# wq2012/SpectralCluster

Measured on AMD Instinct MI355X. Metric: predict() calls/sec, n=8192 d=256 ICASSP2018 (GraphCut, eigengap k in [2,20], cosine k-means), higher is better.
Workload: dtype f64; 1 GPU; icassp2018_graphcut_n8192_d256_k8_max20; n_samples=8192, n_features=256, parallelism=replicas x1, collectives=none

## Files before the change

### spectralcluster_amd/csrc/gemm_f64.hip

```cpp
#include <algorithm>
#include <cstdio>
#include <cstdlib>
#include <type_traits>
#include <vector>

#include <cstring>

#include "sc_internal.h"

namespace sc {

typedef double v4f64 __attribute__((ext_vector_type(4)));
typedef int v4i32 __attribute__((ext_vector_type(4)));
typedef double v2f64 __attribute__((ext_vector_type(2)));

constexpr int BM = 128;
constexpr int BN = 128;
constexpr int BK = 16;

__device__ __forceinline__ int lds_chunk_off(int row, int kc) {
  return row * BK + ((2 * kc) ^ (row & 14));
}

template <bool SYM>
__device__ __forceinline__ void tile_coords(int id, int ntiles_m, int ntiles_n,
                                            int* ti, int* tj) {
  if (SYM) {
    int r = 0, rowlen = ntiles_m;
    while (id >= rowlen) {
      id -= rowlen;
      --rowlen;
      ++r;
    }
    *ti = r;
    *tj = r + id;
  } else {
    *ti = id / ntiles_n;
    *tj = id - (*ti) * ntiles_n;
  }
}

struct GemmStats {
  double* pmax;
  double* psum;
  int mode;
  const double* addend;
};

template <int EPI, bool SYM>
__device__ __forceinline__ void tile_row_stats(const v4f64 (&acc)[4][4], int ti, int tj,
                                               int ntiles, int M, int N, int tid,
                                               const GemmStats& st, double* scratch) {
  const int lane = tid & 63, wave = tid >> 6;
  const int wr = wave >> 1, wc = wave & 1;
  const int li = lane & 15, lg = lane >> 4;
  double* rmax = scratch;
  double* rsum = scratch + 256;
  double* cmax = scratch + 512;
  double* csum = scratch + 768;
  const bool diag_tile = ti == tj;
#pragma unroll
  for (int m = 0; m < 4; ++m) {
#pragma unroll
    for (int r = 0; r < 4; ++r) {
      const int lrow = wr * 64 + m * 16 + lg + 4 * r;
      double mx = -INFINITY, sm = 0.0;
#pragma unroll
      for (int nn = 0; nn < 4; ++nn) {
        const int lcol = wc * 64 + nn * 16 + li;
        const bool inside = tj * BN + lcol < N;
        const bool skip = st.mode == 2 && diag_tile && lrow == lcol;
        double x = acc[m][nn][r];
        if (EPI == kEpiAffinity) x = __builtin_fma(x, 0.5, 0.5);
        if (inside && !skip) mx = fmax(mx, x);
        if (inside) sm += x;
      }
#pragma unroll
      for (int o = 1; o < 16; o <<= 1) {
        mx = fmax(mx, __shfl_xor(mx, o));
        sm += __shfl_xor(sm, o);
      }
      if (li == 0) {
        rmax[wc * 128 + lrow] = mx;
        rsum[wc * 128 + lrow] = sm;
      }
      __builtin_amdgcn_sched_barrier(0);
    }
  }
  if (SYM && !diag_tile) {
#pragma unroll
    for (int nn = 0; nn < 4; ++nn) {
      const int lcol = wc * 64 + nn * 16 + li;
      double mx = -INFINITY, sm = 0.0;
#pragma unroll
      for (int m = 0; m < 4; ++m)
#pragma unroll
        for (int r = 0; r < 4; ++r) {
          const int lrow = wr * 64 + m * 16 + lg + 4 * r;
          double x = acc[m][nn][r];
          if (EPI == kEpiAffinity) x = __builtin_fma(x, 0.5, 0.5);
          if (ti * BM + lrow < M) {
            mx = fmax(mx, x);
            sm += x;
          }
        }
      mx = fmax(mx, __shfl_xor(mx, 16));
      sm += __shfl_xor(sm, 16);
      mx = fmax(mx, __shfl_xor(mx, 32));
      sm += __shfl_xor(sm, 32);
      if (lg == 0) {
        cmax[wr * 128 + lcol] = mx;
        csum[wr * 128 + lcol] = sm;
      }
      __builtin_amdgcn_sched_barrier(0);
    }
  }
  __syncthreads();
  if (tid < 128) {
    const int row = ti * BM + tid;
    if (row < M) {
      st.pmax[(size_t)row * ntiles + tj] = fmax(rmax[tid], rmax[128 + tid]);
      if (st.mode == 1) st.psum[(size_t)row * ntiles + tj] = rsum[tid] + rsum[128 + tid];
    }
  } else if (SYM && !diag_tile) {
    const int c = tid - 128;
    const int row = tj * BN + c;
    if (row < N) {
      st.pmax[(size_t)row * ntiles + ti] = fmax(cmax[c], cmax[128 + c]);
      if (st.mode == 1) st.psum[(size_t)row * ntiles + ti] = csum[c] + csum[128 + c];
    }
  }
}

__device__ __forceinline__ double vmax64(double a, double b) {
  double d;
  asm("v_max_f64 %0, %1, %2" : "=v"(d) : "v"(a), "v"(b));
  return d;
}

constexpr int kEpiColPart = 1024;
constexpr int kEpiStage = 3072;
constexpr int kEpiStageWave = 1280;
constexpr int kEpiRowPitch = 17;

template <int EPI, bool SYM>
__device__ __forceinline__ void tile_row_stats_full(const v4f64 (&acc)[4][4], int ti, int tj,
                                                    int ntiles, int tid, const GemmStats& st,
                                                    double* smem) {
  const int lane = tid & 63, wave = tid >> 6;
  const int wr = wave >> 1, wc = wave & 1;
  const int li = lane & 15, lg = lane >> 4;
  const bool diag_tile = ti == tj;
  const bool sums = st.mode == 1;
  const bool crop = st.mode == 2 && diag_tile && wr == wc;
  double* rmax = smem;
  double* rsum = smem + 256;
  double* cpart = smem + kEpiColPart;
  double* T = smem + kEpiStage + wave * (64 * kEpiRowPitch);
  auto el = [&](int m, int nn, int r) -> double {
    const double x = acc[m][nn][r];
    return EPI == kEpiAffinity ? __builtin_fma(x, 0.5, 0.5) : x;
  };
  auto rows_of = [&](auto is_sum) {
    constexpr bool SUM = decltype(is_sum)::value;
#pragma unroll
    for (int m = 0; m < 4; ++m)
#pragma unroll
      for (int r = 0; r < 4; ++r) {
        double a[4];
#pragma unroll
        for (int nn = 0; nn < 4; ++nn) a[nn] = el(m, nn, r);
        double v;
        if (SUM) {
          v = (a[0] + a[1]) + (a[2] + a[3]);
        } else {
          if (crop && lg + 4 * r == li) a[m] = -INFINITY;
          v = vmax64(vmax64(a[0], a[1]), vmax64(a[2], a[3]));
        }
        T[(m * 16 + lg + 4 * r) * kEpiRowPitch + li] = v;
      }
    __builtin_amdgcn_fence(__ATOMIC_RELEASE, "wavefront");
    __builtin_amdgcn_wave_barrier();
    double t[16];
#pragma unroll
    for (int j = 0; j < 16; ++j) t[j] = T[lane * kEpiRowPitch + j];
#pragma unroll
    for (int w = 8; w >= 1; w >>= 1)
#pragma unroll
      for (int j = 0; j < w; ++j) t[j] = SUM ? t[j] + t[j + w] : vmax64(t[j], t[j + w]);
    (SUM ? rsum : rmax)[wc * 128 + wr * 64 + lane] = t[0];
    __builtin_amdgcn_fence(__ATOMIC_ACQUIRE, "wavefront");
    __builtin_amdgcn_wave_barrier();
  };
  rows_of(std::false_type{});
  if (sums) rows_of(std::true_type{});
  const bool mirror = SYM && !diag_tile;
  if (mirror) {
#pragma unroll
    for (int nn = 0; nn < 4; ++nn) {
      double mx[4], sm[4];
#pragma unroll
      for (int m = 0; m < 4; ++m) {
        const double x0 = el(m, nn, 0), x1 = el(m, nn, 1), x2 = el(m, nn, 2), x3 = el(m, nn, 3);
        mx[m] = vmax64(vmax64(x0, x1), vmax64(x2, x3));
        sm[m] = (x0 + x1) + (x2 + x3);
      }
      const int slot = (wr * 4 + lg) * 128 + wc * 64 + nn * 16 + li;
      cpart[slot] = vmax64(vmax64(mx[0], mx[1]), vmax64(mx[2], mx[3]));
      if (sums) cpart[1024 + slot] = (sm[0] + sm[1]) + (sm[2] + sm[3]);
    }
  }
  __syncthreads();
  if (tid < 128) {
    const size_t at = (size_t)(ti * BM + tid) * ntiles + tj;
    st.pmax[at] = vmax64(rmax[tid], rmax[128 + tid]);
    if (sums) st.psum[at] = rsum[tid] + rsum[128 + tid];
  } else if (mirror) {
    const int c = tid - 128;
    const size_t at = (size_t)(tj * BN + c) * ntiles + ti;
    double t[8];
#pragma unroll
    for (int j = 0; j < 8; ++j) t[j] = cpart[j * 128 + c];
    st.pmax[at] = vmax64(vmax64(vmax64(t[0], t[1]), vmax64(t[2], t[3])),
                         vmax64(vmax64(t[4], t[5]), vmax64(t[6], t[7])));
    if (sums) {
#pragma unroll
      for (int j = 0; j < 8; ++j) t[j] = cpart[1024 + j * 128 + c];
      st.psum[at] = ((t[0] + t[1]) + (t[2] + t[3])) + ((t[4] + t[5]) + (t[6] + t[7]));
    }
  }
}

__global__ void k_gemm_stats_reduce(const double* __restrict__ pmax,
                                    const double* __restrict__ psum, int n, int ntiles,
                                    int mode, double* __restrict__ rowmax,
                                    double* __restrict__ rowsum) {
  const int i = blockIdx.x * blockDim.x + threadIdx.x;
  if (i >= n) return;
  double mx = -INFINITY, sm = 0.0;
  for (int t = 0; t < ntiles; ++t) {
    mx = fmax(mx, pmax[(size_t)i * ntiles + t]);
    if (mode == 1) sm += psum[(size_t)i * ntiles + t];
  }
  if (mode == 2) mx = fmax(mx, 0.0);
  rowmax[i] = mx;
  if (mode == 1) rowsum[i] = sm;
}

constexpr int kStatRows = 32;
constexpr int kStatMaxTiles = 120;
__device__ __forceinline__ void gemm_stats_reduce_lds_body(
    const double* __restrict__ pmax, const double* __restrict__ psum, int n, int ntiles, int mode,
    double* __restrict__ rowmax, double* __restrict__ rowsum) {
  extern __shared__ __attribute__((aligned(16))) double st_smem[];
  const int pitch = ntiles + 1;
  double* lmax = st_smem;
  double* lsum = st_smem + kStatRows * pitch;
  const int r0 = blockIdx.x * kStatRows;
  const int rows = min(kStatRows, n - r0);
  const int total = rows * ntiles;
  for (int e = threadIdx.x; e < total; e += blockDim.x) {
    const int rr = e / ntiles, t = e - rr * ntiles;
    lmax[rr * pitch + t] = pmax[(size_t)r0 * ntiles + e];
    if (mode == 1) lsum[rr * pitch + t] = psum[(size_t)r0 * ntiles + e];
  }
  __syncthreads();
  if ((int)threadIdx.x >= rows) return;
  double mx = -INFINITY, sm = 0.0;
  for (int t = 0; t < ntiles; ++t) {
    mx = fmax(mx, lmax[threadIdx.x * pitch + t]);
    if (mode == 1) sm += lsum[threadIdx.x * pitch + t];
  }
  if (mode == 2) mx = fmax(mx, 0.0);
  rowmax[r0 + threadIdx.x] = mx;
  if (mode == 1) rowsum[r0 + threadIdx.x] = sm;
}
__global__ __launch_bounds__(256) void k_gemm_stats_reduce_lds(
    const double* __restrict__ pmax, const double* __restrict__ psum, int n, int ntiles, int mode,
    double* __restrict__ rowmax, double* __restrict__ rowsum) {
  gemm_stats_reduce_lds_body(pmax, psum, n, ntiles, mode, rowmax, rowsum);
}

struct GemmMember {
  const double* A;
  double* C;
  double* pmax;
  double* psum;
  const int2* tilemap;
  int lda, ldc, n, K, nt;
};
struct GemmGroup {
  GemmMember m[kGroupMax];
  int first[kGroupMax + 1];
};
struct GemmPairMember {
  const double* A;
  const double* B;
  const double* addend;
  double* C;
  const int2* tilemap;
  int lda, ldb, ldc, n, nt;
};
struct GemmPairGroup {
  GemmPairMember m[kGroupMax];
  int first[kGroupMax + 1];
};

constexpr int kEdgePrio = 3;

template <int EPI, bool SYM, bool GROUPED, class GRP>
__device__ __forceinline__ void gemm_nt_body(const double* __restrict__ A,
                                                 int lda,
                                                 const double* __restrict__ B,
                                                 int ldb, double* __restrict__ C,
                                                 int ldc, int M, int N, int K,
                                                 int ntiles_m, int ntiles_n,
                                                 int full_tiles, int ksplit_tail,
                                                 double* __restrict__ partial,
                                                 double* __restrict__ probe_out,
                                                 const int2* __restrict__ tilemap,
                                                 int xcd_chunk, GemmStats stats,
                                                 int* __restrict__ queue,
                                                 int nunits, int persist,
                                                 const GRP* __restrict__ grp) {
  __shared__ __attribute__((aligned(16))) double smem[2 * BM * BK + 2 * BN * BK];
  double(*As)[BM * BK] = reinterpret_cast<double(*)[BM * BK]>(smem);
  double(*Bs)[BN * BK] = reinterpret_cast<double(*)[BN * BK]>(smem + 2 * BM * BK);

  for (int iter = 0;; ++iter) {
  if (iter > 0) {
    if (GROUPED || !persist || queue == nullptr) break;
    __syncthreads();
  }
  if (kEdgePrio & 1) __builtin_amdgcn_s_setprio(3);
  int ti, tj;
  int item_blk = (int)blockIdx.x;
  if constexpr (GROUPED) {
    item_blk = (item_blk & 7) * xcd_chunk + (item_blk >> 3);
    if (item_blk >= grp->first[kGroupMax]) continue;
    int z = 0;
    while (item_blk >= grp->first[z + 1]) ++z;
    const auto& g = grp->m[z];
    item_blk -= grp->first[z];
    C = g.C;
    ldc = g.ldc;
    M = N = g.n;
    ntiles_m = ntiles_n = g.nt;
    tilemap = g.tilemap;
    if constexpr (std::is_same<GRP, GemmPairGroup>::value) {
      A = g.A;
      B = g.B;
      lda = g.lda;
      ldb = g.ldb;
      K = g.n;
      stats.addend = g.addend;
    } else {
      A = B = g.A;
      lda = ldb = g.lda;
      K = g.K;
      stats.pmax = g.pmax;
      stats.psum = g.psum;
    }
  }
  if (queue != nullptr) {
    int* s_item = reinterpret_cast<int*>(smem);
    if (threadIdx.x == 0) {
      const int x = (int)blockIdx.x & 7;
      auto draw = [&](int* counter, int limit) -> int {
        if (__hip_atomic_load(counter, __ATOMIC_RELAXED, __HIP_MEMORY_SCOPE_AGENT) >= limit)
          return -1;
        const int v = __hip_atomic_fetch_add(counter, 1, __ATOMIC_RELAXED,
                                             __HIP_MEMORY_SCOPE_AGENT);
        return v < limit ? v : -1;
      };
      int got = -1;
      {
        const int k = draw(&queue[x], xcd_chunk);
        if (k >= 0) got = x + 8 * k;
      }
      if (got < 0) {
        const int u = draw(&queue[9], nunits);
        if (u >= 0) got = full_tiles + u;
      }
      for (int dx = 1; got < 0 && dx < 8; ++dx) {
        const int xx = (x + dx) & 7;
        const int k = draw(&queue[xx], xcd_chunk);
        if (k >= 0) got = xx + 8 * k;
      }
      *s_item = got;
    }
    __syncthreads();
    item_blk = *s_item;
    __syncthreads();
    if (item_blk < 0) break;
  }
  const bool whole = item_blk < full_tiles;
  const int unit = whole ? 0 : item_blk - full_tiles;
  const int ksplit = whole ? 1 : ksplit_tail;
  const int chunk = unit % ksplit;
  int tile = whole ? item_blk : full_tiles + unit / ksplit;
  if (!GROUPED && whole && xcd_chunk > 0) tile = (tile & 7) * xcd_chunk + (tile >> 3);
  if (!whole) stats.mode = 0;
  if (tilemap != nullptr) {
    const int2 t = tilemap[tile];
    ti = t.x;
    tj = t.y;
  } else {
    tile_coords<SYM>(tile, ntiles_m, ntiles_n, &ti, &tj);
  }
  const int row0 = ti * BM;
  const int col0 = tj * BN;

  int tid_ = threadIdx.x;
  asm volatile("" : "+v"(tid_));
  const int tid = tid_;
  const int lane = tid & 63;
  const int wave = tid >> 6;
  const int wr = wave >> 1;
  const int wc = wave & 1;
  const int li = lane & 15;
  const int lg = lane >> 4;
  long long clk0 = 0, wall0 = 0;
  const bool probe = whole && probe_out != nullptr;
  if (probe) {
    clk0 = clock64();
    wall0 = wall_clock64();
  }
// ... 10 lines not shown
    boff[q] = (unsigned)(((size_t)rb_ * ldb + 2 * kc0) * sizeof(double));
    lds_off[q] = lds_chunk_off(r, kc0);
  }

  v4f64 acc[4][4];
#pragma unroll
  for (int m = 0; m < 4; ++m)
#pragma unroll
    for (int nn = 0; nn < 4; ++nn) acc[m][nn] = (v4f64){0.0, 0.0, 0.0, 0.0};

  const int ktiles_all = (K + BK - 1) / BK;
  const int kper = (ktiles_all + ksplit - 1) / ksplit;
  const int kt_begin = chunk * kper;
  const int kt_end = min(ktiles_all, kt_begin + kper);
  double2 ra[4], rb[4];

  const __amdgpu_buffer_rsrc_t arsrc =
      __builtin_amdgcn_make_buffer_rsrc(const_cast<double*>(A + (size_t)row0 * lda), 0, -1,
                                        0x00020000);
  const __amdgpu_buffer_rsrc_t brsrc =
      __builtin_amdgcn_make_buffer_rsrc(const_cast<double*>(B + (size_t)col0 * ldb), 0, -1,
                                        0x00020000);
  auto gload = [&](int kt) {
    const int koff = kt * BK * (int)sizeof(double);
#pragma unroll
    for (int q = 0; q < 4; ++q) {
      const v4i32 va = __builtin_amdgcn_raw_buffer_load_b128(arsrc, aoff[q], koff, 0);
      const v4i32 vb = __builtin_amdgcn_raw_buffer_load_b128(brsrc, boff[q], koff, 0);
      ra[q] = __builtin_bit_cast(double2, va);
      rb[q] = __builtin_bit_cast(double2, vb);
    }
  };

  auto lds_store = [&](int buf, int kt) {
    const int k0 = kt * BK;
    if (k0 + BK > K) {
      const int k = k0 + 2 * kc0;
#pragma unroll
      for (int q = 0; q < 4; ++q) {
        if (k >= K) { ra[q].x = 0.0; rb[q].x = 0.0; }
        if (k + 1 >= K) { ra[q].y = 0.0; rb[q].y = 0.0; }
      }
    }
#pragma unroll
    for (int q = 0; q < 4; ++q) {
      *reinterpret_cast<double2*>(&As[buf][lds_off[q]]) = ra[q];
      *reinterpret_cast<double2*>(&Bs[buf][lds_off[q]]) = rb[q];
    }
  };

  const int arow = (wr * 64 + li) * BK;
  const int brow = (wc * 64 + li) * BK;

  const int first_buf = (__builtin_amdgcn_s_getreg(6 | (31 << 11)) & 0xfff) != 0 ? 1 : 0;
  if (kt_begin < kt_end) {
    gload(kt_begin);
    lds_store(first_buf, kt_begin);
    if (kt_begin + 1 < kt_end) gload(kt_begin + 1);
  }
  __syncthreads();

  double2 fa0[4], fb0[4], fa1[4], fb1[4];
  auto load_frags = [&](double2 (&a)[4], double2 (&b)[4], const double* Ac, const double* Bc,
                        int p) {
    const int koff = (2 * (4 * p + lg)) ^ (li & 14);
#pragma unroll
    for (int m = 0; m < 4; ++m)
      a[m] = *reinterpret_cast<const double2*>(Ac + arow + m * 16 * BK + koff);
#pragma unroll
    for (int nn = 0; nn < 4; ++nn)
      b[nn] = *reinterpret_cast<const double2*>(Bc + brow + nn * 16 * BK + koff);
  };
  auto mfma16x = [&](const double2 (&a)[4], const double2 (&b)[4]) {
#pragma unroll
    for (int m = 0; m < 4; ++m)
#pragma unroll
      for (int nn = 0; nn < 4; ++nn)
        acc[m][nn] = __builtin_amdgcn_mfma_f64_16x16x4f64(a[m].x, b[nn].x, acc[m][nn], 0, 0, 0);
  };
  auto mfma16y = [&](const double2 (&a)[4], const double2 (&b)[4]) {
#pragma unroll
    for (int m = 0; m < 4; ++m)
#pragma unroll
      for (int nn = 0; nn < 4; ++nn)
        acc[m][nn] = __builtin_amdgcn_mfma_f64_16x16x4f64(a[m].y, b[nn].y, acc[m][nn], 0, 0, 0);
  };
  if (kt_begin < kt_end) load_frags(fa0, fb0, As[first_buf], Bs[first_buf], 0);
  auto k_tile = [&](int kt, auto cur_c, auto prio_c) {
    constexpr int cur = decltype(cur_c)::value;
    constexpr int prio = decltype(prio_c)::value;
    load_frags(fa1, fb1, As[cur], Bs[cur], 1);
    __builtin_amdgcn_sched_barrier(0);
    __builtin_amdgcn_s_setprio(prio);
    mfma16x(fa0, fb0);
    __builtin_amdgcn_sched_barrier(0);
    if (kt + 1 < kt_end) {
      lds_store(cur ^ 1, kt + 1);
      if (kt + 2 < kt_end) gload(kt + 2);
    }
    __builtin_amdgcn_sched_barrier(0);
    mfma16y(fa0, fb0);
    __builtin_amdgcn_s_setprio(0);
    __builtin_amdgcn_sched_barrier(0);
    __syncthreads();
    if (kt + 1 < kt_end) load_frags(fa0, fb0, As[cur ^ 1], Bs[cur ^ 1], 0);
    __builtin_amdgcn_sched_barrier(0);
    __builtin_amdgcn_s_setprio(prio);
    mfma16x(fa1, fb1);
    mfma16y(fa1, fb1);
    __builtin_amdgcn_s_setprio(0);
    __builtin_amdgcn_sched_barrier(0);
  };
  long long wall_k0 = 0;
  if (probe) wall_k0 = wall_clock64();
  {
    using P0 = std::integral_constant<int, 2>;
    using P1 = std::integral_constant<int, 1>;
    int kt = kt_begin;
    if (first_buf && kt < kt_end) {
      k_tile(kt, std::integral_constant<int, 1>{}, P1{});
      ++kt;
    }
    for (; kt + 1 < kt_end; kt += 2) {
      k_tile(kt, std::integral_constant<int, 0>{}, P0{});
      k_tile(kt + 1, std::integral_constant<int, 1>{}, P1{});
    }
    if (kt < kt_end) k_tile(kt, std::integral_constant<int, 0>{}, P0{});
  }

  if (kEdgePrio & 1) __builtin_amdgcn_s_setprio(3);
  long long wall_k1 = 0;
  if (probe) wall_k1 = wall_clock64();
  if (probe && tid == 0) {
    probe_out[2 * item_blk] = (double)(clock64() - clk0);
    probe_out[2 * item_blk + 1] = (double)(wall_k1 - wall0);
    probe_out[2 * full_tiles + item_blk] = (double)wall0;
    probe_out[3 * full_tiles + item_blk] = (double)(wall_k0 - wall0);
  }
  if (ksplit > 1) {
    double* out = partial + (size_t)unit * (BM * BN);
#pragma unroll
    for (int m = 0; m < 4; ++m)
#pragma unroll
      for (int nn = 0; nn < 4; ++nn)
#pragma unroll
        for (int r = 0; r < 4; ++r)
          out[((m * 4 + nn) * 4 + r) * 256 + tid] = acc[m][nn][r];
    continue;
  }
  const bool mirror = SYM && (ti != tj);
  constexpr bool nt_store = (kEdgePrio & 2) != 0;
  const bool full = row0 + BM <= M && col0 + BN <= N;
  if (stats.mode != 0 || mirror) __syncthreads();
  if (stats.mode != 0) {
    if (full) tile_row_stats_full<EPI, SYM>(acc, ti, tj, ntiles_n, tid, stats, smem);
    else tile_row_stats<EPI, SYM>(acc, ti, tj, ntiles_n, M, N, tid, stats, smem);
    __builtin_amdgcn_sched_barrier(0);
  }
  if (probe && tid == 0) probe_out[4 * full_tiles + item_blk] = (double)(wall_clock64() - wall_k1);
  constexpr int kStagePitch = 20;
  double* stage = smem + kEpiStage + wave * kEpiStageWave;
  if (full) {
    double* cdir = C + (size_t)(row0 + wr * 64 + lg) * ldc + (col0 + wc * 64 + li);
    const double* adir = nullptr;
    if (EPI == kEpiAdd)
      adir = stats.addend + (size_t)(row0 + wr * 64 + lg) * ldc + (col0 + wc * 64 + li);
    double* cmir = C + (size_t)(col0 + wc * 64 + (lane >> 3)) * ldc + (row0 + wr * 64 + 2 * (lane & 7));
    double* stage_w = stage + li * kStagePitch + lg;
    const double* stage_r = stage + (lane >> 3) * kStagePitch + 2 * (lane & 7);
    auto store_full = [&](auto mirror_c) {
      constexpr bool MIRROR = decltype(mirror_c)::value;
#pragma unroll
      for (int m = 0; m < 4; ++m) {
#pragma unroll
        for (int r = 0; r < 4; ++r) {
          const size_t roff = (size_t)(m * 16 + 4 * r) * ldc;
#pragma unroll
          for (int nn = 0; nn < 4; ++nn) {
            double v = acc[m][nn][r];
            if (EPI == kEpiAffinity) v = __builtin_fma(v, 0.5, 0.5);
            if (EPI == kEpiAdd) v += adir[roff + nn * 16];
            if (nt_store) __builtin_nontemporal_store(v, cdir + roff + nn * 16);
            else cdir[roff + nn * 16] = v;
            if (MIRROR) stage_w[nn * 16 * kStagePitch + 4 * r] = v;
          }
        }
        if (MIRROR) {
          __builtin_amdgcn_fence(__ATOMIC_RELEASE, "wavefront");
          __builtin_amdgcn_wave_barrier();
#pragma unroll
          for (int i = 0; i < 8; ++i) {
            const v2f64 v = *reinterpret_cast<const v2f64*>(stage_r + i * 8 * kStagePitch);
            v2f64* dst = reinterpret_cast<v2f64*>(cmir + (size_t)(i * 8) * ldc + m * 16);
            if (nt_store) __builtin_nontemporal_store(v, dst);
            else *dst = v;
          }
          __builtin_amdgcn_fence(__ATOMIC_ACQUIRE, "wavefront");
          __builtin_amdgcn_wave_barrier();
        }
      }
    };
    if (mirror) store_full(std::true_type{});
    else store_full(std::false_type{});
  } else {
#pragma unroll
  for (int m = 0; m < 4; ++m) {
#pragma unroll
    for (int nn = 0; nn < 4; ++nn) {
      const int col = col0 + wc * 64 + nn * 16 + li;
#pragma unroll
      for (int r = 0; r < 4; ++r) {
        const int row = row0 + wr * 64 + m * 16 + lg + 4 * r;
        double v = acc[m][nn][r];
        if (EPI == kEpiAffinity) v = __builtin_fma(v, 0.5, 0.5);
        if (row < M && col < N) {
          if (EPI == kEpiAdd) v += stats.addend[(size_t)row * ldc + col];
          if (nt_store) __builtin_nontemporal_store(v, &C[(size_t)row * ldc + col]);
          else C[(size_t)row * ldc + col] = v;
        }
        if (mirror) stage[(nn * 16 + li) * kStagePitch + lg + 4 * r] = v;
      }
    }
    if (mirror) {
      __builtin_amdgcn_fence(__ATOMIC_RELEASE, "wavefront");
      __builtin_amdgcn_wave_barrier();
#pragma unroll
      for (int i = 0; i < 8; ++i) {
        const int c = i * 8 + (lane >> 3);
        const int j = 2 * (lane & 7);
        const double2 v = *reinterpret_cast<const double2*>(stage + c * kStagePitch + j);
        const int mrow = col0 + wc * 64 + c;
        const int mcol = row0 + wr * 64 + m * 16 + j;
        if (mrow < N) {
          double* dst = C + (size_t)mrow * ldc + mcol;
          if (mcol + 1 < M) {
            if (nt_store) {
              __builtin_nontemporal_store(v.x, dst);
              __builtin_nontemporal_store(v.y, dst + 1);
            } else {
              *reinterpret_cast<double2*>(dst) = v;
            }
          } else if (mcol < M) {
            dst[0] = v.x;
          }
        }
      }
      __builtin_amdgcn_fence(__ATOMIC_ACQUIRE, "wavefront");
      __builtin_amdgcn_wave_barrier();
    }
  }
  }
  if (probe) {
    const long long t_issued = wall_clock64();
    asm volatile("s_waitcnt vmcnt(0)" ::: "memory");
    if (tid == 0) {
      probe_out[5 * full_tiles + item_blk] = (double)(t_issued - wall_k1);
      probe_out[6 * full_tiles + item_blk] = (double)(wall_clock64() - wall_k1);
    }
  }
  }
}

template <int EPI, bool SYM>
__global__ __launch_bounds__(256, 2) void k_gemm_nt(const double* __restrict__ A,
                                                 int lda,
                                                 const double* __restrict__ B,
                                                 int ldb, double* __restrict__ C,
                                                 int ldc, int M, int N, int K,
                                                 int ntiles_m, int ntiles_n,
                                                 int full_tiles, int ksplit_tail,
                                                 double* __restrict__ partial,
                                                 double* __restrict__ probe_out,
                                                 const int2* __restrict__ tilemap,
                                                 int xcd_chunk, GemmStats stats,
                                                 int* __restrict__ queue,
                                                 int nunits, int persist) {
  gemm_nt_body<EPI, SYM, false, GemmGroup>(A, lda, B, ldb, C, ldc, M, N, K, ntiles_m, ntiles_n,
                                           full_tiles, ksplit_tail, partial, probe_out, tilemap,
                                           xcd_chunk, stats, queue, nunits, persist, nullptr);
}
template <int EPI>
__global__ __launch_bounds__(256, 2) void k_gemm_nt_g(const GemmGroup grp, int stats_mode,
                                                     int xcd_chunk) {
  GemmStats stats{nullptr, nullptr, stats_mode, nullptr};
  gemm_nt_body<EPI, true, true, GemmGroup>(nullptr, 0, nullptr, 0, nullptr, 0, 0, 0, 0, 0, 0,
                                           0x7fffffff, 1, nullptr, nullptr, nullptr, xcd_chunk,
                                           stats, nullptr, 0, 0, &grp);
}
template <int EPI>
__global__ __launch_bounds__(256, 2) void k_gemm_nt_pg(const GemmPairGroup grp, int xcd_chunk) {
  GemmStats stats{nullptr, nullptr, 0, nullptr};
  gemm_nt_body<EPI, true, true, GemmPairGroup>(nullptr, 0, nullptr, 0, nullptr, 0, 0, 0, 0, 0, 0,
                                               0x7fffffff, 1, nullptr, nullptr, nullptr,
                                               xcd_chunk, stats, nullptr, 0, 0, &grp);
}
template <int EPI>
__global__ __launch_bounds__(256, 2) void k_gemm_nt_pgf(const GemmPairGroup grp, int xcd_chunk) {
  GemmStats stats{nullptr, nullptr, 0, nullptr};
  gemm_nt_body<EPI, false, true, GemmPairGroup>(nullptr, 0, nullptr, 0, nullptr, 0, 0, 0, 0, 0, 0,
                                                0x7fffffff, 1, nullptr, nullptr, nullptr,
                                                xcd_chunk, stats, nullptr, 0, 0, &grp);
}

struct StatsReduceItem {
  const double* pmax;
  const double* psum;
  double* rowmax;
  double* rowsum;
  int n, nt;
};
__global__ __launch_bounds__(256) void k_gemm_stats_reduce_g(const GroupOf<StatsReduceItem> g,
                                                             int mode) {
  const StatsReduceItem& a = g.s[blockIdx.y];
  if ((int)blockIdx.x * kStatRows >= a.n) return;
  if (a.nt > kStatMaxTiles) {
    const int i = blockIdx.x * kStatRows + threadIdx.x;
    if ((int)threadIdx.x >= kStatRows || i >= a.n) return;
    double mx, sm;
    gemm_stats_fold_row(a.pmax + (size_t)i * a.nt,
                        mode == 1 ? a.psum + (size_t)i * a.nt : nullptr, a.nt, mode, &mx, &sm);
    a.rowmax[i] = mx;
    if (mode == 1) a.rowsum[i] = sm;
    return;
  }
  gemm_stats_reduce_lds_body(a.pmax, a.psum, a.n, a.nt, mode, a.rowmax, a.rowsum);
}

template <int EPI, bool SYM>
__global__ __launch_bounds__(256) void k_gemm_reduce(const double* __restrict__ partial,
                                                     double* __restrict__ C, int ldc,
                                                     int M, int N, int ntiles_m,
                                                     int ntiles_n, int tile_offset,
                                                     int ksplit,
                                                     const int2* __restrict__ tilemap,
                                                     const double* __restrict__ addend) {
  int ti, tj;
  if (tilemap != nullptr) {
    const int2 t = tilemap[tile_offset + blockIdx.x];
    ti = t.x;
    tj = t.y;
  } else {
    tile_coords<SYM>(tile_offset + blockIdx.x, ntiles_m, ntiles_n, &ti, &tj);
  }
  const int tid = threadIdx.x;
  const int lane = tid & 63, wave = tid >> 6;
  const int wr = wave >> 1, wc = wave & 1;
  const int li = lane & 15, lg = lane >> 4;
  const bool mirror = SYM && (ti != tj);
  const double* base = partial + (size_t)blockIdx.x * ksplit * (BM * BN);
  {
    const int m = blockIdx.y >> 2;
    {
      const int nn = blockIdx.y & 3;
      const int col = tj * BN + wc * 64 + nn * 16 + li;
#pragma unroll
      for (int r = 0; r < 4; ++r) {
        const int row = ti * BM + wr * 64 + m * 16 + lg + 4 * r;
        const int slot = ((m * 4 + nn) * 4 + r) * 256 + tid;
        double v = 0.0;
        for (int c = 0; c < ksplit; ++c) v += base[(size_t)c * (BM * BN) + slot];
        if (EPI == kEpiAffinity) v = __builtin_fma(v, 0.5, 0.5);
        if (row < M && col < N) {
          if (EPI == kEpiAdd) v += addend[(size_t)row * ldc + col];
          C[(size_t)row * ldc + col] = v;
          if (mirror) C[(size_t)col * ldc + row] = v;
        }
      }
    }
  }
}

template <bool SYM>
__global__ __launch_bounds__(256) void k_gemm_tail_stats(const double* __restrict__ C, int ldc,
                                                         int M, int N, int ntiles_m,
                                                         int ntiles_n, int tile_base,
                                                         const int2* __restrict__ tilemap,
                                                         GemmStats st) {
  int ti, tj;
  if (tilemap != nullptr) {
    const int2 t = tilemap[tile_base + blockIdx.x];
    ti = t.x;
    tj = t.y;
  } else {
    tile_coords<SYM>(tile_base + blockIdx.x, ntiles_m, ntiles_n, &ti, &tj);
  }
  if (blockIdx.y == 1) {
    if (!SYM || ti == tj) return;
    const int t = ti;
    ti = tj;
    tj = t;
  }
  const int lane = threadIdx.x & 63, wave = threadIdx.x >> 6;
  for (int lr = blockIdx.z * 16 + wave; lr < blockIdx.z * 16 + 16; lr += 4) {
    const int row = ti * BM + lr;
    if (row >= M) break;
    double mx = -INFINITY, sm = 0.0;
#pragma unroll
    for (int h = 0; h < 2; ++h) {
      const int col = tj * BN + lane + 64 * h;
      if (col < N) {
        const double x = C[(size_t)row * ldc + col];
        if (!(st.mode == 2 && row == col)) mx = fmax(mx, x);
        sm += x;
      }
    }
#pragma unroll
    for (int o = 1; o < 64; o <<= 1) {
      mx = fmax(mx, __shfl_xor(mx, o));
      sm += __shfl_xor(sm, o);
    }
    if (lane == 0) {
      st.pmax[(size_t)row * ntiles_n + tj] = mx;
      if (st.mode == 1) st.psum[(size_t)row * ntiles_n + tj] = sm;
    }
  }
}

__global__ void k_gemm_queue_init(int* queue) { queue[threadIdx.x] = 0; }

int gemm_resident_slots() {
  static int slots_dev[16] = {0};
  int dev = 0;
  hipGetDevice(&dev);
  dev = dev < 16 ? dev : 0;
  if (slots_dev[dev] == 0) {
    int per_cu = 0;
    hipDeviceProp_t prop;
    hipGetDeviceProperties(&prop, dev);
    hipOccupancyMaxActiveBlocksPerMultiprocessor(
        &per_cu, reinterpret_cast<const void*>(k_gemm_nt<kEpiNone, true>), 256, 0);
    if (per_cu < 1) per_cu = 1;
    slots_dev[dev] = per_cu * prop.multiProcessorCount;
  }
  return slots_dev[dev];
}
constexpr int kQueueWords = 16;
size_t gemm_splitk_workspace_bytes() {
  return (size_t)gemm_resident_slots() * BM * BN * sizeof(double) + kQueueWords * sizeof(int);
}

template <int EPI, bool SYM>
static void launch_variant(hipStream_t s, const double* A, int lda, const double* B,
                           int ldb, double* C, int ldc, int M, int N, int K,
                           double* splitk_ws, const int2* tilemap, const GemmRowStats* rs,
                           const double* addend) {
  GemmStats stats{nullptr, nullptr, 0, addend};
  if (rs != nullptr && rs->mode != 0) {
    stats.pmax = rs->partial_max;
    stats.psum = rs->partial_sum;
    stats.mode = rs->mode;
  }
  const int tm = (M + BM - 1) / BM;
  const int tn = (N + BN - 1) / BN;
  const int tiles = SYM ? tm * (tm + 1) / 2 : tm * tn;
  const int g_slots = gemm_resident_slots();
  double* g_partial = splitk_ws;
  const int ktiles = (K + BK - 1) / BK;
  int full = (tiles / g_slots) * g_slots;
  int rem = tiles - full;
  int ksplit = 1;
  if (rem > 0) {
    if (splitk_ws != nullptr) {
      ksplit = g_slots / rem;
      ksplit = std::min(ksplit, std::max(1, ktiles / 8));
      if (K <= 512 && full == 0) ksplit = 1;
    }
    if (ksplit < 2) {
      full = tiles;
      rem = 0;
      ksplit = 1;
    }
  }
  {
    const int xcd_chunk = (tilemap != nullptr && full % 8 == 0 && full >= 512) ? full / 8 : 0;
    static double* dbg = nullptr;
    static const char* probe_env = getenv("SC_GEMM_CLOCK");
    if (probe_env != nullptr && dbg == nullptr) (void)hipMalloc(&dbg, sizeof(double) * 7 * 8192);
    double* probe = (full > 0 && full <= 8192) ? dbg : nullptr;
    int* queue = nullptr;
    if (K >= 1024 && xcd_chunk > 0 && rem > 0 && SYM) {
      queue = reinterpret_cast<int*>(splitk_ws + (size_t)g_slots * BM * BN);
      hipLaunchKernelGGL(k_gemm_queue_init, dim3(1), dim3(kQueueWords), 0, s, queue);
    }
    const int persist = queue != nullptr ? 1 : 0;
    const int grid = persist ? std::min(g_slots, full + rem * ksplit) : full + rem * ksplit;
    hipLaunchKernelGGL((k_gemm_nt<EPI, SYM>), dim3(grid), dim3(256), 0, s, A, lda,
                       B, ldb, C, ldc, M, N, K, tm, tn, full, ksplit, g_partial, probe, tilemap,
                       xcd_chunk, stats, queue, rem * ksplit, persist);
    if (probe != nullptr) {
      (void)hipStreamSynchronize(s);
      std::vector<double> h(7 * full);
      (void)hipMemcpy(h.data(), dbg, sizeof(double) * 7 * full, hipMemcpyDeviceToHost);
      if (strcmp(probe_env, "1") != 0) {
        const char* path = probe_env;
        if (FILE* f = fopen(path, "w")) {
          for (int b = 0; b < full; ++b)
            fprintf(f, "%d %.0f %.0f %.0f %.0f %.0f %.0f %.0f\n", b, h[2 * b], h[2 * b + 1],
                    h[2 * full + b], h[3 * full + b], h[4 * full + b], h[5 * full + b],
                    h[6 * full + b]);
          fclose(f);
        }
      }
      double c = 0, w = 0;
      for (int i = 0; i < full; ++i) { c += h[2 * i]; w += h[2 * i + 1]; }
      int rate = 0;
      (void)hipDeviceGetAttribute(&rate, hipDeviceAttributeWallClockRate, 0);
      fprintf(stderr, "gemm clock probe (epilogue %d%s): %d tiles, K %d, shader cycles/tile %.0f "
              "(MFMA-bound minimum %.0f), effective shader clock %.1f MHz, tile time %.1f us\n",
              EPI, SYM ? ", symmetric" : "", full, K, c / full,
              (double)((K + BK - 1) / BK) * 64 * 64 * 2, c / w * rate / 1e3,
              w / full / rate * 1e3);
    }
  }
  if (rem > 0) {
    hipLaunchKernelGGL((k_gemm_reduce<EPI, SYM>), dim3(rem, 16), dim3(256), 0, s, g_partial,
                       C, ldc, M, N, tm, tn, full, ksplit, tilemap, addend);
    if (stats.mode != 0)
      hipLaunchKernelGGL((k_gemm_tail_stats<SYM>), dim3(rem, SYM ? 2 : 1, 8), dim3(256), 0, s, C,
                         ldc, M, N, tm, tn, full, tilemap, stats);
  }
  if (stats.mode != 0) {
    if (tn <= kStatMaxTiles)
      hipLaunchKernelGGL(k_gemm_stats_reduce_lds, dim3((M + kStatRows - 1) / kStatRows), dim3(256),
                         2 * kStatRows * (size_t)(tn + 1) * sizeof(double), s, stats.pmax,
                         stats.psum, M, tn, stats.mode, rs->rowmax, rs->rowsum);
    else
      hipLaunchKernelGGL(k_gemm_stats_reduce, dim3((M + 255) / 256), dim3(256), 0, s, stats.pmax,
                         stats.psum, M, tn, stats.mode, rs->rowmax, rs->rowsum);
  }
}

void gemm_build_sym_tilemap(int nt, std::vector<int2>* out) {
  out->clear();
  const int np = (nt + 7) / 8;
  for (int pi = 0; pi < np; ++pi)
    for (int pj = pi; pj < np; ++pj)
      for (int ti = pi * 8; ti < std::min(nt, pi * 8 + 8); ++ti)
        for (int tj = std::max(ti, pj * 8); tj < std::min(nt, pj * 8 + 8); ++tj)
          out->push_back(make_int2(ti, tj));
}
int gemm_tile_dim(int n) { return (n + BM - 1) / BM; }

void launch_gemm_nt(hipStream_t s, const double* A, int lda, const double* B,
                    int ldb, double* C, int ldc, int M, int N, int K,
                    int epilogue, bool symmetric, double* splitk_ws,
                    const int2* tilemap, const GemmRowStats* rs, const double* addend) {
  if (M <= 0 || N <= 0) return;
#define SC_GEMM_CASE(E, S)                                                                \
  launch_variant<E, S>(s, A, lda, B, ldb, C, ldc, M, N, K, splitk_ws, S ? tilemap : nullptr, \
                       rs, addend)
  if (symmetric) {
    if (epilogue == kEpiAffinity) SC_GEMM_CASE(kEpiAffinity, true);
    else if (epilogue == kEpiAdd) SC_GEMM_CASE(kEpiAdd, true);
    else SC_GEMM_CASE(kEpiNone, true);
  } else {
    if (epilogue == kEpiAffinity) SC_GEMM_CASE(kEpiAffinity, false);
    else if (epilogue == kEpiAdd) SC_GEMM_CASE(kEpiAdd, false);
    else SC_GEMM_CASE(kEpiNone, false);
  }
#undef SC_GEMM_CASE
}

void launch_gemm_nt_group(hipStream_t s, const GemmGroupItem* items, int count, int epilogue,
                          int stats_mode, bool reduce_stats) {
  GemmGroup grp;
  memset(&grp, 0, sizeof(grp));
  GroupOf<StatsReduceItem> red;
  memset(&red, 0, sizeof(red));
  int total = 0, nmax = 0;
  for (int z = 0; z < kGroupMax; ++z) {
    grp.first[z] = total;
    if (z >= count || items[z].n <= 0) continue;
    const GemmGroupItem& it = items[z];
    const int nt = (it.n + BM - 1) / BM;
    grp.m[z] = GemmMember{it.A, it.C, it.partial_max, it.partial_sum, it.tilemap,
                          it.lda, it.ldc, it.n, it.K, nt};
    red.s[z] = StatsReduceItem{it.partial_max, it.partial_sum, it.rowmax, it.rowsum, it.n, nt};
    total += nt * (nt + 1) / 2;
    nmax = std::max(nmax, it.n);
  }
  grp.first[kGroupMax] = total;
  if (total == 0) return;
  const int xcd_chunk = (total + 7) / 8;
  const int grid = 8 * xcd_chunk;
  if (epilogue == kEpiAffinity)
    hipLaunchKernelGGL((k_gemm_nt_g<kEpiAffinity>), dim3(grid), dim3(256), 0, s, grp, stats_mode,
                       xcd_chunk);
  else
    hipLaunchKernelGGL((k_gemm_nt_g<kEpiNone>), dim3(grid), dim3(256), 0, s, grp, stats_mode,
                       xcd_chunk);
  if (stats_mode != 0 && reduce_stats)
    hipLaunchKernelGGL(k_gemm_stats_reduce_g, dim3((nmax + kStatRows - 1) / kStatRows, count),
                       dim3(256),
                       2 * kStatRows * (size_t)(std::min((nmax + BM - 1) / BM, kStatMaxTiles) + 1) *
                           sizeof(double),
                       s, red, stats_mode);
}

void launch_gemm_nt_pair_group(hipStream_t s, const GemmPairItem* items, int count, int epilogue,
                               bool full) {
  GemmPairGroup grp;
  memset(&grp, 0, sizeof(grp));
  int total = 0;
  for (int z = 0; z < kGroupMax; ++z) {
    grp.first[z] = total;
    if (z >= count || items[z].n <= 0) continue;
    const GemmPairItem& it = items[z];
    const int nt = (it.n + BM - 1) / BM;
    const bool self = it.B == nullptr;
    grp.m[z] = GemmPairMember{it.A, self ? it.A : it.B, it.addend, it.C,
                              full ? nullptr : it.tilemap,
                              it.lda, self ? it.lda : it.ldb, it.ldc, it.n, nt};
    total += full ? nt * nt : nt * (nt + 1) / 2;
  }
  grp.first[kGroupMax] = total;
  if (total == 0) return;
  const int xcd_chunk = (total + 7) / 8;
  const int grid = 8 * xcd_chunk;
  if (full) {
    if (epilogue == kEpiAdd)
      hipLaunchKernelGGL((k_gemm_nt_pgf<kEpiAdd>), dim3(grid), dim3(256), 0, s, grp, xcd_chunk);
    else
      hipLaunchKernelGGL((k_gemm_nt_pgf<kEpiNone>), dim3(grid), dim3(256), 0, s, grp, xcd_chunk);
    return;
  }
  if (epilogue == kEpiAdd)
    hipLaunchKernelGGL((k_gemm_nt_pg<kEpiAdd>), dim3(grid), dim3(256), 0, s, grp, xcd_chunk);
  else
    hipLaunchKernelGGL((k_gemm_nt_pg<kEpiNone>), dim3(grid), dim3(256), 0, s, grp, xcd_chunk);
}

}
```

Baseline: 387.4 calls/s.

## Add 512-thread 8-wave f64 GEMM variant for short-K symmetric affinity

Adds a new 8-wave (512-thread) symmetric NT GEMM kernel that splits each 128x128 tile into 2x4 wave subtiles of 64x32. Each wave holds half the accumulators, and the kernel has its own row-max epilogue and mirrored store path. It is dispatched for the affinity epilogue when K <= 512 and row-sum stats are not needed, which is the d=256 affinity GEMM here. The aim is more waves per CU and more latency hiding on a short-K, store-bound GEMM. The cost is more LDS fragment loads per MFMA and extra reduction traffic, and the generic stats helper is templated to handle the new wave layout.

```diff
diff --git a/spectralcluster_amd/csrc/gemm_f64.hip b/spectralcluster_amd/csrc/gemm_f64.hip
--- a/spectralcluster_amd/csrc/gemm_f64.hip
+++ b/spectralcluster_amd/csrc/gemm_f64.hip
@@ -47,17 +47,18 @@
   const double* addend;
 };
 
-template <int EPI, bool SYM>
-__device__ __forceinline__ void tile_row_stats(const v4f64 (&acc)[4][4], int ti, int tj,
+template <int EPI, bool SYM, int NN = 4>
+__device__ __forceinline__ void tile_row_stats(const v4f64 (&acc)[4][NN], int ti, int tj,
                                                int ntiles, int M, int N, int tid,
                                                const GemmStats& st, double* scratch) {
+  constexpr int NWC = 8 / NN, WN = 16 * NN;
   const int lane = tid & 63, wave = tid >> 6;
-  const int wr = wave >> 1, wc = wave & 1;
+  const int wr = wave / NWC, wc = wave % NWC;
   const int li = lane & 15, lg = lane >> 4;
   double* rmax = scratch;
-  double* rsum = scratch + 256;
-  double* cmax = scratch + 512;
-  double* csum = scratch + 768;
+  double* rsum = scratch + NWC * 128;
+  double* cmax = scratch + 2 * NWC * 128;
+  double* csum = cmax + 256;
   const bool diag_tile = ti == tj;
 #pragma unroll
   for (int m = 0; m < 4; ++m) {
@@ -66,8 +67,8 @@
       const int lrow = wr * 64 + m * 16 + lg + 4 * r;
       double mx = -INFINITY, sm = 0.0;
 #pragma unroll
-      for (int nn = 0; nn < 4; ++nn) {
-        const int lcol = wc * 64 + nn * 16 + li;
+      for (int nn = 0; nn < NN; ++nn) {
+        const int lcol = wc * WN + nn * 16 + li;
         const bool inside = tj * BN + lcol < N;
         const bool skip = st.mode == 2 && diag_tile && lrow == lcol;
         double x = acc[m][nn][r];
@@ -89,8 +90,8 @@
   }
   if (SYM && !diag_tile) {
 #pragma unroll
-    for (int nn = 0; nn < 4; ++nn) {
-      const int lcol = wc * 64 + nn * 16 + li;
+    for (int nn = 0; nn < NN; ++nn) {
+      const int lcol = wc * WN + nn * 16 + li;
       double mx = -INFINITY, sm = 0.0;
 #pragma unroll
       for (int m = 0; m < 4; ++m)
@@ -119,10 +120,16 @@
   if (tid < 128) {
     const int row = ti * BM + tid;
     if (row < M) {
-      st.pmax[(size_t)row * ntiles + tj] = fmax(rmax[tid], rmax[128 + tid]);
-      if (st.mode == 1) st.psum[(size_t)row * ntiles + tj] = rsum[tid] + rsum[128 + tid];
-    }
-  } else if (SYM && !diag_tile) {
+      double mx = rmax[tid], sm = rsum[tid];
+#pragma unroll
+      for (int w = 1; w < NWC; ++w) {
+        mx = fmax(mx, rmax[w * 128 + tid]);
+        sm += rsum[w * 128 + tid];
+      }
+      st.pmax[(size_t)row * ntiles + tj] = mx;
+      if (st.mode == 1) st.psum[(size_t)row * ntiles + tj] = sm;
+    }
+  } else if (tid < 256 && SYM && !diag_tile) {
     const int c = tid - 128;
     const int row = tj * BN + c;
     if (row < N) {
@@ -739,6 +746,416 @@
                                                 xcd_chunk, stats, nullptr, 0, 0, &grp);
 }
 
+constexpr int kShortK = 512;
+constexpr int kEpiStageWave8 = 640;
+
+template <int EPI>
+__device__ __forceinline__ void tile_row_max_full8(const v4f64 (&acc)[4][2], int ti, int tj,
+                                                   int ntiles, int tid, const GemmStats& st,
+                                                   double* smem) {
+  const int lane = tid & 63, wave = tid >> 6;
+  const int wr = wave >> 2, wc = wave & 3;
+  const int li = lane & 15, lg = lane >> 4;
+  const bool diag_tile = ti == tj;
+  const bool crop = st.mode == 2 && diag_tile;
+  double* rmax = smem;
+  double* cpart = smem + kEpiColPart;
+  double* T = smem + kEpiStage + wave * kEpiStageWave8;
+  auto el = [&](int m, int nn, int r) -> double { return acc[m][nn][r]; };
+  auto fin = [&](double x) -> double {
+    return EPI == kEpiAffinity ? __builtin_fma(x, 0.5, 0.5) : x;
+  };
+#pragma unroll
+  for (int half = 0; half < 2; ++half) {
+#pragma unroll
+    for (int mm = 0; mm < 2; ++mm) {
+      const int m = 2 * half + mm;
+#pragma unroll
+      for (int r = 0; r < 4; ++r) {
+        double a[2];
+#pragma unroll
+        for (int nn = 0; nn < 2; ++nn) {
+          a[nn] = el(m, nn, r);
+          if (crop && 4 * wr + m == 2 * wc + nn && lg + 4 * r == li) a[nn] = -INFINITY;
+        }
+        T[(mm * 16 + lg + 4 * r) * kEpiRowPitch + li] = vmax64(a[0], a[1]);
+      }
+    }
+    __builtin_amdgcn_fence(__ATOMIC_RELEASE, "wavefront");
+    __builtin_amdgcn_wave_barrier();
+    {
+      double t[8];
+#pragma unroll
+      for (int j = 0; j < 8; ++j) t[j] = T[(lane >> 1) * kEpiRowPitch + (lane & 1) * 8 + j];
+#pragma unroll
+      for (int w = 4; w >= 1; w >>= 1)
+#pragma unroll
+        for (int j = 0; j < w; ++j) t[j] = vmax64(t[j], t[j + w]);
+      const double v = vmax64(t[0], __shfl_xor(t[0], 1));
+      if ((lane & 1) == 0) rmax[wc * 128 + wr * 64 + half * 32 + (lane >> 1)] = v;
+    }
+    __builtin_amdgcn_fence(__ATOMIC_ACQUIRE, "wavefront");
+    __builtin_amdgcn_wave_barrier();
+  }
+  const bool mirror = !diag_tile;
+  if (mirror) {
+#pragma unroll
+    for (int nn = 0; nn < 2; ++nn) {
+      double mx[4];
+#pragma unroll
+      for (int m = 0; m < 4; ++m)
+        mx[m] = vmax64(vmax64(el(m, nn, 0), el(m, nn, 1)), vmax64(el(m, nn, 2), el(m, nn, 3)));
+      cpart[(wr * 4 + lg) * 128 + wc * 32 + nn * 16 + li] =
+          vmax64(vmax64(mx[0], mx[1]), vmax64(mx[2], mx[3]));
+    }
+  }
+  __syncthreads();
+  if (tid < 128) {
+    st.pmax[(size_t)(ti * BM + tid) * ntiles + tj] = fin(
+        vmax64(vmax64(rmax[tid], rmax[128 + tid]), vmax64(rmax[256 + tid], rmax[384 + tid])));
+  } else if (tid < 256 && mirror) {
+    const int c = tid - 128;
+    double t[8];
+#pragma unroll
+    for (int j = 0; j < 8; ++j) t[j] = cpart[j * 128 + c];
+    st.pmax[(size_t)(tj * BN + c) * ntiles + ti] =
+        fin(vmax64(vmax64(vmax64(t[0], t[1]), vmax64(t[2], t[3])),
+                   vmax64(vmax64(t[4], t[5]), vmax64(t[6], t[7]))));
+  }
+}
+
+template <int EPI, bool GROUPED>
+__device__ __forceinline__ void gemm_nt_body8(const double* __restrict__ A, int lda,
+                                              double* __restrict__ C, int ldc, int n, int K,
+                                              int ntiles, int full_tiles, int ksplit_tail,
+                                              double* __restrict__ partial,
+                                              double* __restrict__ probe_out,
+                                              const int2* __restrict__ tilemap, int xcd_chunk,
+                                              GemmStats stats,
+                                              const GemmGroup* __restrict__ grp) {
+  __shared__ __attribute__((aligned(16))) double smem[2 * BM * BK + 2 * BN * BK];
+  double(*As)[BM * BK] = reinterpret_cast<double(*)[BM * BK]>(smem);
+  double(*Bs)[BN * BK] = reinterpret_cast<double(*)[BN * BK]>(smem + 2 * BM * BK);
+  if (kEdgePrio & 1) __builtin_amdgcn_s_setprio(3);
+  int item_blk = (int)blockIdx.x;
+  if constexpr (GROUPED) {
+    item_blk = (item_blk & 7) * xcd_chunk + (item_blk >> 3);
+    if (item_blk >= grp->first[kGroupMax]) return;
+    int z = 0;
+    while (item_blk >= grp->first[z + 1]) ++z;
+    const auto& g = grp->m[z];
+    item_blk -= grp->first[z];
+    A = g.A;
+    lda = g.lda;
+    C = g.C;
+    ldc = g.ldc;
+    n = g.n;
+    K = g.K;
+    ntiles = g.nt;
+    tilemap = g.tilemap;
+    stats.pmax = g.pmax;
+    stats.psum = g.psum;
+  }
+  const bool whole = item_blk < full_tiles;
+  const int unit = whole ? 0 : item_blk - full_tiles;
+  const int ksplit = whole ? 1 : ksplit_tail;
+  const int chunk = unit % ksplit;
+  int tile = whole ? item_blk : full_tiles + unit / ksplit;
+  if (!GROUPED && whole && xcd_chunk > 0) tile = (tile & 7) * xcd_chunk + (tile >> 3);
+  if (!whole) stats.mode = 0;
+  int ti, tj;
+  if (tilemap != nullptr) {
+    const int2 t = tilemap[tile];
+    ti = t.x;
+    tj = t.y;
+  } else {
+    tile_coords<true>(tile, ntiles, ntiles, &ti, &tj);
+  }
+  const int row0 = ti * BM;
+  const int col0 = tj * BN;
+  int tid, lane, wave, wr, wc, li, lg;
+  auto thread_coords = [&]() {
+    tid = threadIdx.x;
+    asm volatile("" : "+v"(tid));
+    lane = tid & 63;
+    wave = tid >> 6;
+    wr = wave >> 2;
+    wc = wave & 3;
+    li = lane & 15;
+    lg = lane >> 4;
+  };
+  thread_coords();
+  long long clk0 = 0, wall0 = 0;
+  const bool probe = whole && probe_out != nullptr;
+  if (probe) {
+    clk0 = clock64();
+    wall0 = wall_clock64();
+  }
+
+  unsigned aoff[2], boff[2];
+  int lds_off[2];
+  const int kc0 = tid & 7;
+#pragma unroll
+  for (int q = 0; q < 2; ++q) {
+    const int r = (tid >> 3) + 64 * q;
+    const int ra_ = row0 + r < n ? r : n - 1 - row0;
+    const int rb_ = col0 + r < n ? r : n - 1 - col0;
+    aoff[q] = (unsigned)(((size_t)ra_ * lda + 2 * kc0) * sizeof(double));
+    boff[q] = (unsigned)(((size_t)rb_ * lda + 2 * kc0) * sizeof(double));
+    lds_off[q] = lds_chunk_off(r, kc0);
+  }
+  v4f64 acc[4][2];
+#pragma unroll
+  for (int m = 0; m < 4; ++m)
+#pragma unroll
+    for (int nn = 0; nn < 2; ++nn) acc[m][nn] = (v4f64){0.0, 0.0, 0.0, 0.0};
+
+  const int ktiles_all = (K + BK - 1) / BK;
+  const int kper = (ktiles_all + ksplit - 1) / ksplit;
+  const int kt_begin = chunk * kper;
+  const int kt_end = min(ktiles_all, kt_begin + kper);
+  double2 ra[2], rb[2];
+  const __amdgpu_buffer_rsrc_t arsrc = __builtin_amdgcn_make_buffer_rsrc(
+      const_cast<double*>(A + (size_t)row0 * lda), 0, -1, 0x00020000);
+  const __amdgpu_buffer_rsrc_t brsrc = __builtin_amdgcn_make_buffer_rsrc(
+      const_cast<double*>(A + (size_t)col0 * lda), 0, -1, 0x00020000);
+  auto gload = [&](int kt) {
+    const int koff = kt * BK * (int)sizeof(double);
+#pragma unroll
+    for (int q = 0; q < 2; ++q) {
+      const v4i32 va = __builtin_amdgcn_raw_buffer_load_b128(arsrc, aoff[q], koff, 0);
+      const v4i32 vb = __builtin_amdgcn_raw_buffer_load_b128(brsrc, boff[q], koff, 0);
+      ra[q] = __builtin_bit_cast(double2, va);
+      rb[q] = __builtin_bit_cast(double2, vb);
+    }
+  };
+  auto lds_store = [&](int buf, int kt) {
+    const int k0 = kt * BK;
+    if (k0 + BK > K) {
+      const int k = k0 + 2 * kc0;
+#pragma unroll
+      for (int q = 0; q < 2; ++q) {
+        if (k >= K) { ra[q].x = 0.0; rb[q].x = 0.0; }
+        if (k + 1 >= K) { ra[q].y = 0.0; rb[q].y = 0.0; }
+      }
+    }
+#pragma unroll
+    for (int q = 0; q < 2; ++q) {
+      *reinterpret_cast<double2*>(&As[buf][lds_off[q]]) = ra[q];
+      *reinterpret_cast<double2*>(&Bs[buf][lds_off[q]]) = rb[q];
+    }
+  };
+  const int arow = (wr * 64 + li) * BK;
+  const int brow = (wc * 32 + li) * BK;
+  if (kt_begin < kt_end) {
+    gload(kt_begin);
+    lds_store(0, kt_begin);
+    if (kt_begin + 1 < kt_end) gload(kt_begin + 1);
+  }
+  __syncthreads();
+
+  double2 fa[4], fb[2];
+  auto load_frags = [&](const double* Ac, const double* Bc, int p) {
+    const int koff = (2 * (4 * p + lg)) ^ (li & 14);
+#pragma unroll
+    for (int m = 0; m < 4; ++m)
+      fa[m] = *reinterpret_cast<const double2*>(Ac + arow + m * 16 * BK + koff);
+#pragma unroll
+    for (int nn = 0; nn < 2; ++nn)
+      fb[nn] = *reinterpret_cast<const double2*>(Bc + brow + nn * 16 * BK + koff);
+  };
+  auto mfma_half = [&]() {
+#pragma unroll
+    for (int m = 0; m < 4; ++m)
+#pragma unroll
+      for (int nn = 0; nn < 2; ++nn)
+        acc[m][nn] = __builtin_amdgcn_mfma_f64_16x16x4f64(fa[m].x, fb[nn].x, acc[m][nn], 0, 0, 0);
+#pragma unroll
+    for (int m = 0; m < 4; ++m)
+#pragma unroll
+      for (int nn = 0; nn < 2; ++nn)
+        acc[m][nn] = __builtin_amdgcn_mfma_f64_16x16x4f64(fa[m].y, fb[nn].y, acc[m][nn], 0, 0, 0);
+  };
+  if (kt_begin < kt_end) load_frags(As[0], Bs[0], 0);
+  auto k_tile = [&](int kt, auto cur_c) {
+    constexpr int cur = decltype(cur_c)::value;
+    __builtin_amdgcn_s_setprio(1);
+    mfma_half();
+    __builtin_amdgcn_s_setprio(0);
+    __builtin_amdgcn_sched_barrier(0);
+    load_frags(As[cur], Bs[cur], 1);
+    if (kt + 1 < kt_end) {
+      lds_store(cur ^ 1, kt + 1);
+      if (kt + 2 < kt_end) gload(kt + 2);
+    }
+    __builtin_amdgcn_sched_barrier(0);
+    __syncthreads();
+    __builtin_amdgcn_s_setprio(1);
+    mfma_half();
+    __builtin_amdgcn_s_setprio(0);
+    __builtin_amdgcn_sched_barrier(0);
+    if (kt + 1 < kt_end) load_frags(As[cur ^ 1], Bs[cur ^ 1], 0);
+    __builtin_amdgcn_sched_barrier(0);
+  };
+  long long wall_k0 = 0;
+  if (probe) wall_k0 = wall_clock64();
+  {
+    int kt = kt_begin;
+    for (; kt + 1 < kt_end; kt += 2) {
+      k_tile(kt, std::integral_constant<int, 0>{});
+      k_tile(kt + 1, std::integral_constant<int, 1>{});
+    }
+    if (kt < kt_end) k_tile(kt, std::integral_constant<int, 0>{});
+  }
+
+  if (kEdgePrio & 1) __builtin_amdgcn_s_setprio(3);
+  thread_coords();
+  long long wall_k1 = 0;
+  if (probe) wall_k1 = wall_clock64();
+  if (probe && tid == 0) {
+    probe_out[2 * item_blk] = (double)(clock64() - clk0);
+    probe_out[2 * item_blk + 1] = (double)(wall_k1 - wall0);
+    probe_out[2 * full_tiles + item_blk] = (double)wall0;
+    probe_out[3 * full_tiles + item_blk] = (double)(wall_k0 - wall0);
+  }
+  if (ksplit > 1) {
+    double* out = partial + (size_t)unit * (BM * BN) + ((wr * 2 + (wc >> 1)) * 64 + lane);
+#pragma unroll
+    for (int m = 0; m < 4; ++m)
+#pragma unroll
+      for (int nn = 0; nn < 2; ++nn)
+#pragma unroll
+        for (int r = 0; r < 4; ++r)
+          out[((m * 4 + 2 * (wc & 1) + nn) * 4 + r) * 256] = acc[m][nn][r];
+    return;
+  }
+  const bool mirror = ti != tj;
+  constexpr bool nt_store = (kEdgePrio & 2) != 0;
+  const bool full = row0 + BM <= n && col0 + BN <= n;
+  if (stats.mode != 0 || mirror) __syncthreads();
+  if (stats.mode != 0) {
+    if (full) tile_row_max_full8<EPI>(acc, ti, tj, ntiles, tid, stats, smem);
+    else tile_row_stats<EPI, true, 2>(acc, ti, tj, ntiles, n, n, tid, stats, smem);
+    __builtin_amdgcn_sched_barrier(0);
+  }
+  if (probe && tid == 0) probe_out[4 * full_tiles + item_blk] = (double)(wall_clock64() - wall_k1);
+  constexpr int kStagePitch = 20;
+  double* stage = smem + kEpiStage + wave * kEpiStageWave8;
+  if (full) {
+    double* cdir = C + (size_t)(row0 + wr * 64 + lg) * ldc + (col0 + wc * 32 + li);
+    double* cmir = C + (size_t)(col0 + wc * 32 + (lane >> 3)) * ldc + (row0 + wr * 64 + 2 * (lane & 7));
+    double* stage_w = stage + li * kStagePitch + lg;
+    const double* stage_r = stage + (lane >> 3) * kStagePitch + 2 * (lane & 7);
+    auto store_full = [&](auto mirror_c) {
+      constexpr bool MIRROR = decltype(mirror_c)::value;
+#pragma unroll
+      for (int m = 0; m < 4; ++m) {
+#pragma unroll
+        for (int r = 0; r < 4; ++r) {
+          const size_t roff = (size_t)(m * 16 + 4 * r) * ldc;
+#pragma unroll
+          for (int nn = 0; nn < 2; ++nn) {
+            double v = acc[m][nn][r];
+            if (EPI == kEpiAffinity) v = __builtin_fma(v, 0.5, 0.5);
+            if (nt_store) __builtin_nontemporal_store(v, cdir + roff + nn * 16);
+            else cdir[roff + nn * 16] = v;
+            if (MIRROR) stage_w[nn * 16 * kStagePitch + 4 * r] = v;
+          }
+        }
+        if (MIRROR) {
+          __builtin_amdgcn_fence(__ATOMIC_RELEASE, "wavefront");
+          __builtin_amdgcn_wave_barrier();
+#pragma unroll
+          for (int i = 0; i < 4; ++i) {
+            const v2f64 v = *reinterpret_cast<const v2f64*>(stage_r + i * 8 * kStagePitch);
+            v2f64* dst = reinterpret_cast<v2f64*>(cmir + (size_t)(i * 8) * ldc + m * 16);
+            if (nt_store) __builtin_nontemporal_store(v, dst);
+            else *dst = v;
+          }
+          __builtin_amdgcn_fence(__ATOMIC_ACQUIRE, "wavefront");
+          __builtin_amdgcn_wave_barrier();
+        }
+      }
+    };
+    if (mirror) store_full(std::true_type{});
+    else store_full(std::false_type{});
+  } else {
+#pragma unroll
+    for (int m = 0; m < 4; ++m) {
+#pragma unroll
+      for (int nn = 0; nn < 2; ++nn) {
+        const int col = col0 + wc * 32 + nn * 16 + li;
+#pragma unroll
+        for (int r = 0; r < 4; ++r) {
+          const int row = row0 + wr * 64 + m * 16 + lg + 4 * r;
+          double v = acc[m][nn][r];
+          if (EPI == kEpiAffinity) v = __builtin_fma(v, 0.5, 0.5);
+          if (row < n && col < n) {
+            if (nt_store) __builtin_nontemporal_store(v, &C[(size_t)row * ldc + col]);
+            else C[(size_t)row * ldc + col] = v;
+          }
+          if (mirror) stage[(nn * 16 + li) * kStagePitch + lg + 4 * r] = v;
+        }
+      }
+      if (mirror) {
+        __builtin_amdgcn_fence(__ATOMIC_RELEASE, "wavefront");
+        __builtin_amdgcn_wave_barrier();
+#pragma unroll
+        for (int i = 0; i < 4; ++i) {
+          const int c = i * 8 + (lane >> 3);
+          const int j = 2 * (lane & 7);
+          const double2 v = *reinterpret_cast<const double2*>(stage + c * kStagePitch + j);
+          const int mrow = col0 + wc * 32 + c;
+          const int mcol = row0 + wr * 64 + m * 16 + j;
+          if (mrow < n) {
+            double* dst = C + (size_t)mrow * ldc + mcol;
+            if (mcol + 1 < n) {
+              if (nt_store) {
+                __builtin_nontemporal_store(v.x, dst);
+                __builtin_nontemporal_store(v.y, dst + 1);
+              } else {
+                *reinterpret_cast<double2*>(dst) = v;
+              }
+            } else if (mcol < n) {
+              dst[0] = v.x;
+            }
+          }
+        }
+        __builtin_amdgcn_fence(__ATOMIC_ACQUIRE, "wavefront");
+        __builtin_amdgcn_wave_barrier();
+      }
+    }
+  }
+  if (probe) {
+    const long long t_issued = wall_clock64();
+    asm volatile("s_waitcnt vmcnt(0)" ::: "memory");
+    if (tid == 0) {
+      probe_out[5 * full_tiles + item_blk] = (double)(t_issued - wall_k1);
+      probe_out[6 * full_tiles + item_blk] = (double)(wall_clock64() - wall_k1);
+    }
+  }
+}
+
+template <int EPI>
+__global__ __launch_bounds__(512, 4) void k_gemm_nt8(const double* __restrict__ A, int lda,
+                                                     double* __restrict__ C, int ldc, int n,
+                                                     int K, int ntiles, int full_tiles,
+                                                     int ksplit_tail,
+                                                     double* __restrict__ partial,
+                                                     double* __restrict__ probe_out,
+                                                     const int2* __restrict__ tilemap,
+                                                     int xcd_chunk, GemmStats stats) {
+  gemm_nt_body8<EPI, false>(A, lda, C, ldc, n, K, ntiles, full_tiles, ksplit_tail, partial,
+                            probe_out, tilemap, xcd_chunk, stats, nullptr);
+}
+template <int EPI>
+__global__ __launch_bounds__(512, 4) void k_gemm_nt_g8(const GemmGroup grp, int stats_mode,
+                                                       int xcd_chunk) {
+  GemmStats stats{nullptr, nullptr, stats_mode, nullptr};
+  gemm_nt_body8<EPI, true>(nullptr, 0, nullptr, 0, 0, 0, 0, 0x7fffffff, 1, nullptr, nullptr,
+                           nullptr, xcd_chunk, stats, &grp);
+}
+
 struct StatsReduceItem {
   const double* pmax;
   const double* psum;
@@ -921,9 +1338,17 @@
     }
     const int persist = queue != nullptr ? 1 : 0;
     const int grid = persist ? std::min(g_slots, full + rem * ksplit) : full + rem * ksplit;
-    hipLaunchKernelGGL((k_gemm_nt<EPI, SYM>), dim3(grid), dim3(256), 0, s, A, lda,
-                       B, ldb, C, ldc, M, N, K, tm, tn, full, ksplit, g_partial, probe, tilemap,
-                       xcd_chunk, stats, queue, rem * ksplit, persist);
+    bool short_k = false;
+    if constexpr (EPI == kEpiAffinity && SYM) {
+      short_k = K <= kShortK && A == B && lda == ldb && M == N && stats.mode != 1;
+      if (short_k)
+        hipLaunchKernelGGL((k_gemm_nt8<EPI>), dim3(grid), dim3(512), 0, s, A, lda, C, ldc, M, K,
+                           tm, full, ksplit, g_partial, probe, tilemap, xcd_chunk, stats);
+    }
+    if (!short_k)
+      hipLaunchKernelGGL((k_gemm_nt<EPI, SYM>), dim3(grid), dim3(256), 0, s, A, lda,
+                         B, ldb, C, ldc, M, N, K, tm, tn, full, ksplit, g_partial, probe, tilemap,
+                         xcd_chunk, stats, queue, rem * ksplit, persist);
     if (probe != nullptr) {
       (void)hipStreamSynchronize(s);
       std::vector<double> h(7 * full);
@@ -1004,11 +1429,12 @@
   memset(&grp, 0, sizeof(grp));
   GroupOf<StatsReduceItem> red;
   memset(&red, 0, sizeof(red));
-  int total = 0, nmax = 0;
+  int total = 0, nmax = 0, kmax = 0;
   for (int z = 0; z < kGroupMax; ++z) {
     grp.first[z] = total;
     if (z >= count || items[z].n <= 0) continue;
     const GemmGroupItem& it = items[z];
+    kmax = std::max(kmax, it.K);
     const int nt = (it.n + BM - 1) / BM;
     grp.m[z] = GemmMember{it.A, it.C, it.partial_max, it.partial_sum, it.tilemap,
                           it.lda, it.ldc, it.n, it.K, nt};
@@ -1020,7 +1446,10 @@
   if (total == 0) return;
   const int xcd_chunk = (total + 7) / 8;
   const int grid = 8 * xcd_chunk;
-  if (epilogue == kEpiAffinity)
+  if (epilogue == kEpiAffinity && kmax <= kShortK && stats_mode != 1)
+    hipLaunchKernelGGL((k_gemm_nt_g8<kEpiAffinity>), dim3(grid), dim3(512), 0, s, grp, stats_mode,
+                       xcd_chunk);
+  else if (epilogue == kEpiAffinity)
     hipLaunchKernelGGL((k_gemm_nt_g<kEpiAffinity>), dim3(grid), dim3(256), 0, s, grp, stats_mode,
                        xcd_chunk);
   else
```

Result: slower. 382.9 calls/s (-1.2%).
